# Qualcomm-AI-research/FP8-quantization

Measured on AMD Instinct MI355X. Metric: FP8 quant+dequant Gelems/sec, higher is better.
Workload: dtype f32; 1 GPU; conv1-shaped weights [2097152,3,7,7] fp32 per GPU, per-channel E5M2 quantize+dequantize, fixed ranges from current_minmax (BASELINE config 2, synthetic NxCxKxK scale-up); elements_per_gpu=308281344, parallelism=1 GPU

## Files before the change

fp8-quantization_amd/csrc/fp8q_common.h:

```cpp
#pragma once
#include <hip/hip_runtime.h>
#include <math.h>

#include <atomic>
#include <stdint.h>
#include <stdio.h>
#include <stdlib.h>
#include <string.h>

#include <climits>
#include <type_traits>

#include "../../include/fp8q.h"
#include "fp8q_device.h"

using namespace fp8q;

constexpr int FP8Q_CODEC_NOT_FLAT = -1000;
int fp8q_codec_flat_launch(bool encode, const void *in, void *out, int64_t C, int64_t inner, const float *maxval,
                           const QFmt &f, int n_bits, hipStream_t st);

namespace {

constexpr int kUnroll = 4;
constexpr int kTargetBlocks = 2048;
constexpr int kDirectMaxInner = 16384;
constexpr int kDirectElems = 32768;
static const int64_t kNtBytes = [] {
    const char *e = getenv("FP8Q_NT_MB");
    const long v = e ? atol(e) : 0;
    return (int64_t)(v >= 1 ? v : 64) << 20;
}();

inline int env_int(const char *name, int dflt, int lo = INT_MIN, int hi = INT_MAX)
{
    const char *e = getenv(name);
    if (!e) return dflt;
    const long v = atol(e);
    return v < lo ? lo : (v > hi ? hi : (int)v);
}

template <auto V>
using Const = std::integral_constant<decltype(V), V>;
// ... 233 lines not shown
```

fp8-quantization_amd/csrc/fp8q_quant.hip:

```cpp
#include "fp8q_rows.h"
#include "fp8q_select.h"

namespace {

template <bool NT, int U>
__device__ __forceinline__ void quant_rows_body(const float *__restrict__ x, float *__restrict__ y, int64_t inner,
                                                const float *__restrict__ maxval, int per_channel, const QFmt &f)
{
    __shared__ float2 lut[kLutMax];
    const int row = blockIdx.y;
    const int tid = threadIdx.x;
    const Chan cfull = make_chan(maxval[per_channel ? row : 0], f);
    for (int i = tid; i <= f.pmax; i += kBlock) lut[i] = lut_entry(cfull, i, f.M);
    __syncthreads();
    const ChanLite c = lite(cfull);
    const float pmaxf = (float)f.pmax;
    const float qthr = f.qthr;

    const float *xr = x + (int64_t)row * inner;
    float *yr = y + (int64_t)row * inner;
    int64_t head = ((16 - ((uintptr_t)xr & 15)) & 15) >> 2;
    if (head > inner) head = inner;
    const int64_t nvec = (inner - head) >> 2;
    const int64_t tail0 = head + (nvec << 2);
// ... 202 lines not shown
    for (int64_t row = (int64_t)blockIdx.x * (kBlock / 64) + wave; row < C; row += (int64_t)gridDim.x * (kBlock / 64)) {
        const Chan cfull = make_chan(maxval[row], f);
        for (int i = lane; i <= f.pmax; i += 64) lut[wave][i] = lut_entry(cfull, i, f.M);
        __builtin_amdgcn_wave_barrier();
        const ChanLite c = lite(cfull);
        const float *xr = x + row * inner;
        float *yr = y + row * inner;
        for (int i = lane; i < inner; i += 64) yr[i] = quant_one(xr[i], c, lut[wave], pmaxf, f.qthr);
        __builtin_amdgcn_wave_barrier();
    }
}

template <class SEL>
__global__ void __launch_bounds__(kBlock)
k_quant_scalar_dm(const float *__restrict__ x, float *__restrict__ y, int64_t inner, const float *__restrict__ maxval,
                  int per_channel, SEL sel)
{
    const QFmt f = pick_fmt(sel);
    quant_scalar_body(x, y, inner, maxval, per_channel, f);
}

template <bool NT>
__global__ void __launch_bounds__(kBlock)
k_copy(const vf4 *__restrict__ x, vf4 *__restrict__ y, int64_t nvec)
{
    const int tid = threadIdx.x;
    const int64_t step = (int64_t)gridDim.x * (kBlock * kUnroll);
    for (int64_t base = (int64_t)blockIdx.x * (kBlock * kUnroll); base < nvec; base += step) {
        if (base + kBlock * kUnroll <= nvec) {
            vf4 v[kUnroll];
#pragma unroll
            for (int u = 0; u < kUnroll; ++u) v[u] = ld16<NT>(x + base + u * kBlock + tid);
#pragma unroll
            for (int u = 0; u < kUnroll; ++u) st16<NT>(y + base + u * kBlock + tid, v[u]);
        } else {
            for (int u = 0; u < kUnroll; ++u) {
                const int64_t i = base + u * kBlock + tid;
                if (i < nvec) st16<NT>(y + i, ld16<NT>(x + i));
            }
        }
    }
}

struct RowGrid {
    bool nt;
    bool small;
    int64_t bx;
    int64_t bs;
};

constexpr int64_t kSmallElems = (int64_t)8 << 20;

inline int64_t k1_total_cap(bool nt, int64_t pieces, int64_t big_cap = 65536)
{
    return (!nt || pieces <= 4096) ? kTargetBlocks : big_cap;
}

template <class CapRule>
RowGrid row_grid(int64_t C, int64_t inner, int64_t small_elems, CapRule total_cap, bool partial_piece = false)
{
    RowGrid g;
// ... 190 lines not shown
    const bool aligned = (((uintptr_t)x ^ (uintptr_t)y) & 15) == 0 && ((uintptr_t)x & 3) == 0;
    if (!aligned) return FP8Q_EUNSUPPORTED;
    SelIn si;
    si.mses = mses;
    si.grid = grid;
    si.n_m = n_m;
    si.n_cand = n_cand;
    si.so = *so;
    static const int64_t sel_cap = getenv("FP8Q_SEL_CAP") ? atoll(getenv("FP8Q_SEL_CAP")) : kTargetBlocks;
    const RowGrid g = row_grid(1, n, kSmallElems, [](bool nt, int64_t pieces) { return k1_total_cap(nt, pieces, sel_cap); });
    dispatch_k1(g, [&](auto NT, auto U) {
        hipLaunchKernelGGL((k_quant_rows_sel<NT(), U()>), dim3((unsigned)g.bx, 1u), dim3(kBlock), 0, st, x, y, n, sel, si);
    });
    return launch_rc();
}

extern "C" {

int fp8q_copy_f32(const float *x, float *y, int64_t n, fp8q_stream_t stream)
{
    if (!x || !y || n < 0 || (n & 3) || ((uintptr_t)x & 15) || ((uintptr_t)y & 15)) return FP8Q_EINVAL;
    if (n == 0) return FP8Q_OK;
    const RowGrid g = row_grid(1, n, 0, [](bool, int64_t pieces) { return (int64_t)(pieces > 4096 ? 65536 : kTargetBlocks); }, true);
    dispatch<true, false>(g.nt, [&](auto NT) {
        hipLaunchKernelGGL(k_copy<NT()>, dim3((unsigned)g.bx), dim3(kBlock), 0, (hipStream_t)stream, (const vf4 *)x, (vf4 *)y, n / 4);
    });
    return launch_rc();
}

}
```

fp8-quantization_amd/csrc/fp8q_rows.h:

```cpp
#pragma once
#include "fp8q_common.h"

namespace {

constexpr int kModeQuant = 0, kModeFused = 1, kModeMinMax = 2;
constexpr int kModeEncode = 3, kModeDecode = 4;

struct TileArgs {
    int inner;
    int rows;
    int lut_stride;
    int group;
    int coaligned;
    uint32_t magic;
    uint32_t lmagic;
};

__device__ __forceinline__ ChanLite lite_lds(const Chan *c)
{
    const float4 h = *reinterpret_cast<const float4 *>(c);
    ChanLite l;
    l.maxv = h.x;
    l.minv = h.y;
    l.bias = h.z;
    l.pthr = h.w;
    return l;
}

constexpr int kChunkElems = 4096, kChunkGroups = 1024, kFlatMaxCh = 8;
constexpr int kFlatFusedMaxInner = 256;

struct FlatArgs {
    int inner;
    int rpc;
    int nch;
    int lut_stride;
    int group;
    int tail;
    uint32_t magic;
    uint32_t rmagic;
    int64_t nvec;
    int64_t nchunks;
    int n_bits;
    int pad0;
};

struct __attribute__((aligned(16))) ChunkInfo {
    int64_t row_lo;
    int phase;
    int nrows;
    int len;
    int tail;
    int pad[2];
};

__device__ __forceinline__ int64_t div_rows(int64_t elo, int inner)
{
    int64_t q = (int64_t)((double)elo / (double)inner);
    int64_t r = elo - q * inner;
    if (r < 0) --q, r += inner;
    if (r >= inner) ++q;
    return q;
}

constexpr int kNotFlat = -1000;
static_assert(kNotFlat == FP8Q_CODEC_NOT_FLAT, "fp8q_codec_flat_launch passes the code through");

inline int64_t flat_rpc(int64_t inner) { return (inner + (kChunkElems + 3) - 2) / inner + 1; }

inline int64_t flat_per_row(int lut_stride, bool fused = false) { return 16 + 16 + (int64_t)lut_stride * 8 + (fused ? 4 : 0); }

inline FlatArgs flat_geometry(int64_t C, int64_t inner, int lut_stride)
{
    FlatArgs a = {};
    a.inner = (int)inner;
    a.lut_stride = lut_stride;
    a.magic = magic_of((int)inner);
    const int64_t n = C * inner;
    a.nvec = n >> 2;
    a.tail = (int)(n & 3);
    a.nchunks = cdiv(a.nvec, kChunkGroups);
    a.rpc = (int)flat_rpc(inner);
    a.rmagic = magic_of(a.rpc);
    return a;
}

}

#define FP8Q_HIDDEN extern "C" __attribute__((visibility("hidden")))
FP8Q_HIDDEN int64_t fp8q_direct_max_inner();
FP8Q_HIDDEN int fp8q_launch_rows_direct(int mode, const float *x, float *y, int64_t C, int64_t inner, const float *maxval,
                                   float *row_min, float *row_max, float *maxval_out, const QFmt &f, const FoldArgs &fa,
                                   hipStream_t st);
FP8Q_HIDDEN int fp8q_launch_rows_reg(bool quant, const float *x, float *y, int64_t C, int64_t inner, float *row_min, float *row_max,
                                float *maxval_out, const QFmt &f, const FoldArgs &fa, hipStream_t st);
FP8Q_HIDDEN int fp8q_launch_rows_staged_mm(const float *x, int64_t C, int64_t inner, float *row_min, float *row_max,
                                      float *maxval_out, const FoldArgs &fa, hipStream_t st);
```

fp8-quantization_amd/csrc/fp8q_rows.hip:

```cpp
#include "fp8q_rows.h"

namespace {

template <int MODE, bool LUT, bool NT>
__global__ void __launch_bounds__(kBlock, 4)
k_rows_direct(const float *__restrict__ x, float *__restrict__ y, int64_t C,
              const float *__restrict__ maxval, float *row_min, float *row_max, float *maxval_out,
              QFmt f, TileArgs a, FoldArgs fa)
{
    extern __shared__ __attribute__((aligned(16))) unsigned char smem[];
    const int Rmax = a.rows;
    float *rowmv = reinterpret_cast<float *>(smem);
    float4 *patch = reinterpret_cast<float4 *>(rowmv + ((Rmax + 3) & ~3));
    Chan *chans = reinterpret_cast<Chan *>(patch + Rmax);
    float2 *lut = reinterpret_cast<float2 *>(chans + Rmax);
    const int tid = threadIdx.x;
    constexpr int BS = kBlock;
    const int G = a.group, rpp = BS / G;
    const int sub = tid & (G - 1), slot = tid / G;
    const int inner = a.inner, inner4 = inner & ~3;
    const float pmaxf = (float)f.pmax;
    __shared__ double ftab_lds[kFastTabSize];
    const double *ftab = ftab_lds;
    if (MODE != kModeMinMax)
// ... 100 lines not shown
                    const int ch = div_small((uint32_t)o, a.magic);
                    const int b = inner - (o - ch * inner);
                    float e[4] = {v[u].x, v[u].y, v[u].z, v[u].w};
                    if (LUT) {
                        quant_group<4>(e, lite_lds(chans + ch), lut + ch * a.lut_stride, pmaxf, f.qthr);
                    } else {
                        const Chan c = chans[ch];
#pragma unroll
                        for (int q = 0; q < 4; ++q) e[q] = quant_direct(e[q], c, f.M);
                    }
                    if (b < 4) {
                        const float4 pt = patch[ch];
                        e[3] = b == 3 ? pt.x : (b == 2 ? pt.y : pt.z);
                        if (b < 3) e[2] = b == 2 ? pt.x : pt.y;
                        if (b < 2) e[1] = pt.x;
                    }
                    st16u<NT>(yt + o, vf4{e[0], e[1], e[2], e[3]});
                }
            }
        }
    }
}

template <int MODE, bool NT>
__global__ void __launch_bounds__(kBlock, 4)
k_rows_flat(const float *__restrict__ x, float *__restrict__ y, const float *__restrict__ maxval,
            float *row_min, float *row_max, float *maxval_out, QFmt f, FlatArgs a)
{
    extern __shared__ __attribute__((aligned(16))) unsigned char smem[];
    __shared__ double ftab[kFastTabSize];
    const int Rt = a.rpc * a.nch;
    ChunkInfo *cinfo = reinterpret_cast<ChunkInfo *>(smem);
    float4 *patch = reinterpret_cast<float4 *>(cinfo + kFlatMaxCh);
    float4 *chl = patch + Rt;
    float2 *lut = reinterpret_cast<float2 *>(chl + Rt);
    float *rowmv = reinterpret_cast<float *>(lut + Rt * a.lut_stride);
    const int tid = threadIdx.x;
    const int inner = a.inner;
    const int64_t G = gridDim.x;
    const float pmaxf = (float)f.pmax;
    for (int i = tid; i < kFastTabSize; i += kBlock) ftab[i] = kFastTab[i];

    for (int64_t c0 = blockIdx.x; c0 < a.nchunks; c0 += G * a.nch) {
        int nct = 1;
        while (nct < a.nch && c0 + nct * G < a.nchunks) ++nct;
        const int nlr = nct * a.rpc;
        __syncthreads();
        if (tid < nct) {
            const int64_t c = c0 + tid * G;
            const int64_t elo = c * kChunkElems;
            const int64_t rem = a.nvec * 4 - elo;
            ChunkInfo ci;
            ci.len = rem < kChunkElems ? (int)rem : kChunkElems;
            ci.tail = (c == a.nchunks - 1) ? a.tail : 0;
            ci.row_lo = elo / inner;
            ci.phase = (int)(elo - ci.row_lo * inner);
            ci.nrows = (ci.phase + ci.len + ci.tail - 1) / inner + 1;
            ci.pad[0] = ci.pad[1] = 0;
            cinfo[tid] = ci;
        }
        __syncthreads();
        if (MODE == kModeFused) {
            const int Gl = a.group, rpp = kBlock / Gl, sub = tid & (Gl - 1), slot = tid / Gl;
            const int inner4 = inner & ~3;
            for (int lrb = 0; lrb < nlr; lrb += rpp) {
                const int lr = lrb + slot;
                const int i = div_small((uint32_t)lr, a.rmagic), r = lr - i * a.rpc;
                const bool valid = lr < nlr && r < cinfo[i].nrows;
                MinMax m;
                mm_init(m);
                if (valid) {
                    const float *xr = x + (cinfo[i].row_lo + r) * inner;
                    int j = sub * 4;
                    for (; j + 3 * Gl * 4 < inner4; j += Gl * 16) {
                        vf4 v[4];
#pragma unroll
                        for (int u = 0; u < 4; ++u) v[u] = ld16u<false>(xr + j + u * Gl * 4);
#pragma unroll
                        for (int u = 0; u < 4; ++u) {
                            mm_acc(m, v[u].x);
                            mm_acc(m, v[u].y);
                            mm_acc(m, v[u].z);
                            mm_acc(m, v[u].w);
                        }
// ... 157 lines not shown
                const int o = phase + 4 * q;
                const int lrow = div_small((uint32_t)o, a.magic);
                const int b = inner - (o - lrow * inner);
                const int lr = lr0 + lrow;
                float e[4] = {v[u].x, v[u].y, v[u].z, v[u].w};
                quant_group<4>(e, lite_of(chl[lr]), lut + lr * a.lut_stride, pmaxf, f.qthr);
                if (b < 4) {
                    const float4 pt = patch[lr];
                    e[3] = b == 3 ? pt.x : (b == 2 ? pt.y : pt.z);
                    if (b < 3) e[2] = b == 2 ? pt.x : pt.y;
                    if (b < 2) e[1] = pt.x;
                }
                st16<NT>(yv + q, vf4{e[0], e[1], e[2], e[3]});
            }
        }
    }
}

constexpr int kStagePad = 256;
constexpr int kStageWin = kStagePad + kChunkElems + kStagePad;
constexpr size_t kStageMaxLds = 36 * 1024;
constexpr int kStageGrid = 2048;
static_assert(kStagePad >= kFlatFusedMaxInner - 1 && kStagePad % 4 == 0, "border rows must fit the pads");

__device__ __forceinline__ ChunkInfo stage_geometry(int64_t c, const FlatArgs &a)
{
    ChunkInfo ci;
    const int64_t elo = c * kChunkElems;
    const int64_t rem = a.nvec * 4 - elo;
    ci.len = rem < kChunkElems ? (int)rem : kChunkElems;
    ci.tail = (c == a.nchunks - 1) ? a.tail : 0;
    ci.row_lo = div_rows(elo, a.inner);
    ci.phase = (int)(elo - ci.row_lo * a.inner);
    ci.nrows = div_small((uint32_t)(ci.phase + ci.len + ci.tail - 1), a.magic) + 1;
    ci.pad[0] = ci.nrows * a.inner - ci.phase - ci.len;
    ci.pad[1] = 0;
    return ci;
}

__device__ __forceinline__ ChunkInfo stage_geometry_next(const ChunkInfo &cur, int64_t cn, uint32_t adv, const FlatArgs &a)
{
    ChunkInfo ci;
    const int64_t elo = cn * kChunkElems;
    const int64_t rem = a.nvec * 4 - elo;
    ci.len = rem < kChunkElems ? (int)rem : kChunkElems;
    ci.tail = (cn == a.nchunks - 1) ? a.tail : 0;
    const uint32_t t = (uint32_t)cur.phase + adv;
    const uint32_t q = (uint32_t)div_small(t, a.magic);
    ci.row_lo = cur.row_lo + q;
    ci.phase = (int)(t - q * (uint32_t)a.inner);
    ci.nrows = div_small((uint32_t)(ci.phase + ci.len + ci.tail - 1), a.magic) + 1;
    ci.pad[0] = ci.nrows * a.inner - ci.phase - ci.len;
    ci.pad[1] = 0;
    return ci;
}

constexpr int kStageU = 4;

template <bool NT>
__device__ __forceinline__ void stage_load_body(const float *x, int64_t c, const FlatArgs &a, vf4 (&v)[kStageU])
{
// ... 250 lines not shown

}

int64_t fp8q_direct_max_inner()
{
    static const int v = [] {
        const char *e = getenv("FP8Q_DIRECT_MAX_INNER");
        const int n = e ? atoi(e) : 0;
        return n >= 4 && n <= kDirectMaxInner ? n : 2047;
    }();
    return v;
}

static int64_t flat_nch(const FlatArgs &a, int64_t per_row, int64_t lds_bytes, int64_t max_nch)
{
    int64_t nch = (lds_bytes - (int64_t)kFlatMaxCh * sizeof(ChunkInfo)) / (a.rpc * per_row);
    if (nch > max_nch) nch = max_nch;
    while (nch > 1 && cdiv(a.nchunks, nch) < 1024) --nch;
    return nch;
}

static size_t flat_shmem(const FlatArgs &a, int64_t per_row) { return (size_t)kFlatMaxCh * sizeof(ChunkInfo) + (size_t)a.rpc * a.nch * per_row; }

static int launch_rows_flat(int mode, const float *x, float *y, int64_t C, int64_t inner, const float *maxval,
                            float *row_min, float *row_max, float *maxval_out, const QFmt &f, hipStream_t st)
{
    static const int flat_env = env_int("FP8Q_FLAT", 1);
    if (!flat_env || mode == kModeMinMax || inner < 4) return kNotFlat;
    if ((((uintptr_t)x | (uintptr_t)y) & 15) != 0) return kNotFlat;
    if (mode == kModeFused && (inner > kFlatFusedMaxInner || x == y)) return kNotFlat;
    FlatArgs a = flat_geometry(C, inner, f.pmax + 1);
    const int64_t per_row = flat_per_row(a.lut_stride, mode == kModeFused);
    static const int lds_kb_env = [] {
        const char *e = getenv("FP8Q_FLAT_LDS_KB");
        const int v = e ? atoi(e) : 0;
        return v >= 4 && v <= 120 ? v : 36;
    }();
    static const int nch_env = [] {
        const char *e = getenv("FP8Q_FLAT_NCH");
        const int v = e ? atoi(e) : 0;
        return v >= 1 && v <= kFlatMaxCh ? v : 4;
    }();
    const int64_t nch = flat_nch(a, per_row, (int64_t)lds_kb_env * 1024, nch_env);
    if (nch < 1) return kNotFlat;
    const bool nt = C * inner * 4 >= kNtBytes;
    if (mode == kModeFused) {
        static const int staged_env = env_int("FP8Q_STAGED", 1);
        static const int staged_grid = [] {
            const char *e = getenv("FP8Q_STAGED_GRID");
            const int v = e ? atoi(e) : -1;
            return v >= 0 ? v : kStageGrid;
        }();
        const size_t sh = (size_t)kStageWin * sizeof(float) + (size_t)a.rpc * per_row;
        if (staged_env && sh <= kStageMaxLds) {
            int gs = 0;
            while (gs < 6 && (2 << gs) * a.rpc <= kBlock) ++gs;
            a.group = gs;
            a.nch = 1;
            const int64_t blocks = staged_grid ? balanced_blocks(a.nchunks, staged_grid) : a.nchunks;
            dispatch<true, false>(nt, [&](auto NT) {
                hipLaunchKernelGGL((k_rows_staged<NT()>), dim3((unsigned)blocks), dim3(kBlock), sh, st, x, y, row_min, row_max,
                                   maxval_out, f, a);
            });
            return launch_rc();
        }
    }
    a.nch = (int)nch;
    int G = 1;
    while (G < 64 && (int64_t)G * 24 < inner) G <<= 1;
    a.group = G;
    static const int grid_env = env_int("FP8Q_FLAT_GRID", 0, 0);
    int64_t blocks = cdiv(a.nchunks, a.nch);
    const int64_t grid_cap = grid_env ? grid_env : ((mode == kModeQuant && a.nchunks <= 16384) ? 1024 : 32768);
    if (blocks > grid_cap) blocks = grid_cap;
    dispatch<kModeQuant, kModeFused>(mode, [&](auto MODE) {
        dispatch<true, false>(nt, [&](auto NT) {
            hipLaunchKernelGGL((k_rows_flat<MODE(), NT()>), dim3((unsigned)blocks), dim3(kBlock), flat_shmem(a, per_row), st, x, y,
                               maxval, row_min, row_max, maxval_out, f, a);
        });
    });
    return launch_rc();
}

__attribute__((visibility("hidden"))) int fp8q_codec_flat_launch(bool encode, const void *in, void *out, int64_t C,
                                                                 int64_t inner, const float *maxval, const QFmt &f,
                                                                 int n_bits, hipStream_t st)
{
    const void *fp = encode ? in : (const void *)out;
    const void *cp = encode ? (const void *)out : in;
    if (inner < 4 || inner > fp8q_direct_max_inner() || ((uintptr_t)fp & 15) != 0 || ((uintptr_t)cp & 3) != 0) return kNotFlat;
    FlatArgs a = flat_geometry(C, inner, f.pmax + 1);
    a.n_bits = n_bits;
    const int64_t per_row = flat_per_row(a.lut_stride);
    const int64_t nch = flat_nch(a, per_row, 36 * 1024, 4);
    if (nch < 1) return kNotFlat;
    a.nch = (int)nch;
    a.group = 1;
    int64_t blocks = cdiv(a.nchunks, nch);
    if (blocks > 32768) blocks = 32768;
    const bool nt = C * inner * 4 >= kNtBytes;
    const float *xf = (const float *)in;
    float *yf = (float *)out;
    dispatch<kModeEncode, kModeDecode>(encode ? kModeEncode : kModeDecode, [&](auto MODE) {
        dispatch<true, false>(nt, [&](auto NT) {
            hipLaunchKernelGGL((k_rows_flat<MODE(), NT()>), dim3((unsigned)blocks), dim3(kBlock), flat_shmem(a, per_row), st, xf, yf,
                               maxval, nullptr, nullptr, nullptr, f, a);
        });
    });
    return launch_rc();
}

int fp8q_launch_rows_staged_mm(const float *x, int64_t C, int64_t inner, float *row_min, float *row_max, float *maxval_out,
                          const FoldArgs &fa, hipStream_t st)
{
    static const int staged_env = env_int("FP8Q_STAGED", 1);
    if (!staged_env || inner < 4 || inner > kFlatFusedMaxInner || ((uintptr_t)x & 15) != 0) return kNotFlat;
    FlatArgs a = flat_geometry(C, inner, 0);
    int gs = 0;
    while (gs < 3 && (2 << gs) * a.rpc <= kBlock) ++gs;
    a.group = gs;
    static const int grid_env = env_int("FP8Q_STAGED_MM_GRID", 0, 0);
    const int64_t blocks = grid_env ? balanced_blocks(a.nchunks, grid_env) : a.nchunks;
    dispatch<true, false>(C * inner * 4 >= kNtBytes, [&](auto NT) {
        hipLaunchKernelGGL((k_rows_staged_mm<NT()>), dim3((unsigned)blocks), dim3(kBlock), 0, st, x, row_min, row_max, maxval_out,
                           fa, a);
    });
// ... 49 lines not shown
    static const int mm_blocks_env = env_int("FP8Q_K2_BLOCKS", 65536);
    const int64_t bcap = mode == kModeMinMax ? mm_blocks_env : 2 * kTargetBlocks;
    if (blocks > bcap) blocks = balanced_blocks(blocks, bcap);
    const bool nt = C * inner * 4 >= kNtBytes;
    const dim3 g((unsigned)blocks), b(BSZ);
    auto launch = [&](auto MODE, auto LUT, auto NT) {
        hipLaunchKernelGGL((k_rows_direct<MODE(), LUT(), NT()>), g, b, shmem, st, x, y, C, maxval, row_min, row_max,
                           maxval_out, f, a, fa);
    };
    if (mode == kModeMinMax) {
        launch(Const<kModeMinMax>{}, Const<false>{}, Const<false>{});
    } else {
        dispatch<kModeQuant, kModeFused>(mode, [&](auto MODE) {
            dispatch<true, false>(lut, [&](auto LUT) { dispatch<true, false>(nt, [&](auto NT) { launch(MODE, LUT, NT); }); });
        });
    }
    return launch_rc();
}

extern "C" {

int64_t fp8q_fused_max_inner(void) { return kDirectMaxInner; }

int fp8q_minmax_quantize_f32(const float *x, float *y, int64_t C, int64_t inner, float *row_min,
                             float *row_max, float *maxval_out, float mbits, int n_bits,
                             int sign_bits, fp8q_stream_t stream)
{
    if (C < 0 || inner < 0) return FP8Q_EINVAL;
    QFmt f;
    if (int rc = make_fmt(mbits, n_bits, sign_bits, &f)) return rc;
    if (C == 0 || inner == 0) return FP8Q_OK;
    if (!x || !y) return FP8Q_EINVAL;
    if (inner > kDirectMaxInner) return FP8Q_ETOOLONG;
    if (((uintptr_t)x & 3) != 0 || ((uintptr_t)y & 3) != 0) return FP8Q_EINVAL;
    hipStream_t st = (hipStream_t)stream;
    static const bool small_fused = env_int("FP8Q_SMALL_FUSED", 1) != 0;
    const FoldArgs nofold = {0, 1, 0.0f, 0.0f};
    if (small_fused && C * inner <= kSmallFusedElems && inner <= kSmallFusedInner) {
        dispatch<1, 2, 3, 4, 8>((int)cdiv(inner, 64), [&](auto EPL) {
            hipLaunchKernelGGL(k_small_rows_fused<EPL()>, dim3((unsigned)cdiv(C, kBlock / 64)), dim3(kBlock), 0, st, x, y, C,
                               (int)inner, row_min, row_max, maxval_out, f);
        });
        return launch_rc();
    }
    const int rc = fp8q_launch_rows_reg(true, x, y, C, inner, row_min, row_max, maxval_out, f, nofold, st);
    if (rc != kNotFlat) return rc;
// ... 5 lines not shown
```

fp8-quantization_amd/fp8q/_lib.py:

```python
import ctypes
import os

from . import build as _build

_lib = None

_i64 = ctypes.c_int64
_vp = ctypes.c_void_p
_f = ctypes.c_float
_i = ctypes.c_int



class MseState(ctypes.Structure):
    _fields_ = [("cur_min", _vp), ("cur_max", _vp), ("absmax", _vp), ("grid", _vp), ("mses", _vp), ("maxval", _vp),
                ("xmin", _vp), ("mbits", _vp), ("vote", _vp)]


class MseRouteInfo(ctypes.Structure):
    _fields_ = [("kernel", _i), ("finish", _i), ("nsplit", _i64), ("tiles_per_wg", _i), ("part_wgs", _i), ("slice_min", _i),
                ("moments_threads", _i), ("n_superblocks", _i64), ("top_scan", _i), ("reserved", _i)]


class AffinePre(ctypes.Structure):
    _fields_ = [("x", _vp), ("residual", _vp), ("alpha_beta", _vp), ("N", _i64), ("C", _i64), ("HW", _i64), ("act", _i)]


class AffineRouteInfo(ctypes.Structure):
    _fields_ = [("kernel", _i), ("direct", _i), ("cpp", _i), ("launches", _i), ("grid_x", _i64), ("grid_y", _i64)]


class MxtRouteInfo(ctypes.Structure):
    _fields_ = [("kernel", _i), ("tile_rows", _i), ("tile_cols", _i), ("nontemporal", _i), ("code_store_bytes", _i),
                ("reserved", _i)]


class TensorDesc(ctypes.Structure):
    _fields_ = [("x", _vp), ("y", _vp), ("maxval", _vp), ("C", _i64), ("inner", _i64), ("n_maxval", _i64),
                ("mbits", _f), ("n_bits", _i), ("sign_bits", _i)]


SIGNATURES = {
    "fp8q_version": (_i, []),
    "fp8q_strerror": (ctypes.c_char_p, [_i]),
    "fp8q_quantize_f32": (_i, [_vp, _vp, _i64, _i64, _vp, _i64, _f, _i, _i, _vp]),
    "fp8q_minmax_workspace_bytes": (ctypes.c_size_t, [_i64, _i64]),
    "fp8q_minmax_f32": (_i, [_vp, _i64, _i64, _vp, _vp, _vp, _i, ctypes.c_double, _i, _vp,
                             ctypes.c_size_t, _vp]),
    "fp8q_minmax_packed_f32": (_i, [_vp, _i64, _i64, _vp, _vp, _vp, _vp, _i, ctypes.c_double, _i, _vp,
                                    ctypes.c_size_t, _vp]),
    "fp8q_ranges_unpack_f32": (_i, [_vp, _i64, _vp, _vp, _vp, _vp]),
    "fp8q_minmax_workspace_check": (_i, [_vp, ctypes.c_size_t, _i, _vp]),
    "fp8q_fused_max_inner": (_i64, []),
    "fp8q_minmax_quantize_f32": (_i, [_vp, _vp, _i64, _i64, _vp, _vp, _vp, _f, _i, _i, _vp]),
    "fp8q_mse_workspace_bytes": (ctypes.c_size_t, [_i64, _i64, _i64, _i]),
    "fp8q_mse_grid_f32": (_i, [_vp, _i64, _i64, _vp, _i64, ctypes.POINTER(_f), _i, _i, _i, _vp, _vp,
                               ctypes.c_size_t, _vp]),
# ... 24 lines not shown
    "fp8q_quantizer_prepare_f32": (_i, [_vp, _f, _i, _i, _vp, _vp]),
    "fp8q_affine_act_quantize_ab_f32": (_i, [_vp, _vp, _vp, _i64, _i64, _i64, _vp, _i, _vp, _vp, _f, _i, _i, _vp]),
    "fp8q_affine_act_f32": (_i, [_vp, _vp, _vp, _i64, _i64, _i64, _vp, _i, _vp]),
    "fp8q_affine_act_route": (_i, [_i64, _i64, _i64, _i, ctypes.POINTER(AffineRouteInfo)]),
    "fp8q_affine_act_minmax_linspace_f32": (_i, [_vp, _vp, _vp, _i64, _i64, _i64, _vp, _i, _vp, _vp, _vp, _vp, _i, ctypes.c_double,
                                                 ctypes.c_double, _vp, ctypes.c_size_t, _vp]),
    "fp8q_affine_act_minmax_workspace_bytes": (ctypes.c_size_t, [_i64, _i64, _i64]),
    "fp8q_affine_act_minmax_f32": (_i, [_vp, _vp, _i64, _i64, _i64, _vp, _vp, _vp, _vp, _i, _vp, _vp, _vp, _i,
                                        ctypes.c_double, _i, _vp, ctypes.c_size_t, _vp]),
    "fp8q_affine_act_minmax_packed_f32": (_i, [_vp, _vp, _i64, _i64, _i64, _vp, _vp, _vp, _vp, _i, _vp, _vp, _vp, _vp,
                                               _i, ctypes.c_double, _i, _vp, ctypes.c_size_t, _vp]),
    "fp8q_encode_u8": (_i, [_vp, _vp, _i64, _i64, _vp, _i64, _f, _i, _i, _vp]),
    "fp8q_decode_u8": (_i, [_vp, _vp, _i64, _i64, _vp, _i64, _f, _i, _i, _vp]),
    "fp8q_multi_quantize_f32": (_i, [ctypes.POINTER(TensorDesc), _i, _vp]),
    "fp8q_multi_minmax_quantize_f32": (_i, [ctypes.POINTER(TensorDesc), ctypes.POINTER(_vp), _i, _vp]),
    "fp8q_multi_encode_u8": (_i, [ctypes.POINTER(TensorDesc), _i, _vp]),
    "fp8q_multi_minmax_encode_u8": (_i, [ctypes.POINTER(TensorDesc), ctypes.POINTER(_vp), _i, _vp]),
    "fp8q_multi_decode_u8": (_i, [ctypes.POINTER(TensorDesc), _i, _vp]),
    "fp8q_multi_plan_create": (_i, [ctypes.POINTER(TensorDesc), _i, ctypes.POINTER(_vp)]),
    "fp8q_multi_plan_launch": (_i, [_vp, _vp]),
    "fp8q_multi_plan_launches": (_i, [_vp]),
    "fp8q_multi_plan_destroy": (None, [_vp]),
    "fp8q_copy_f32": (_i, [_vp, _vp, _i64, _vp]),
    "fp8q_int_quantize_f32": (_i, [_vp, _vp, _i64, _i64, _vp, _vp, _i64, _vp, _i, _i, _f, _vp]),
    "fp8q_int_set_range_f32": (_i, [_vp, _vp, _i64, _vp, _vp, _vp, _i, _i, _f, _vp]),
    "fp8q_int_range_quantize_f32": (_i, [_vp, _vp, _i64, _i64, _vp, _vp, _i64, _vp, _vp, _vp, _i, _i, _f, _vp]),
    "fp8q_int_minmax_quantize_f32": (_i, [_vp, _vp, _i64, _i64, _vp, _vp, _vp, _vp, _vp, _i, _i, _f, _vp,
                                          ctypes.c_size_t, _vp]),
    "fp8q_int_affine_act_quantize_f32": (_i, [_vp, _vp, _vp, _i64, _i64, _i64, _vp, _i, _vp, _vp, _vp, _i, _i, _f, _vp]),
    "fp8q_int_affine_act_range_quantize_f32": (_i, [_vp, _vp, _vp, _i64, _i64, _i64, _vp, _i, _vp, _vp, _vp, _vp, _vp, _i, _i,
                                                    _f, _vp]),
    "fp8q_int_sse_grid_workspace_bytes": (ctypes.c_size_t, [_i64, _i64, _i64]),
    "fp8q_int_sse_grid_f32": (_i, [_vp, _i64, _i64, _vp, _i64, _i, _i, _i, _f, _vp, _vp, ctypes.c_size_t, _vp]),
    "fp8q_int_sse_grid_f64": (_i, [_vp, _i64, _i64, _vp, _i64, _i, _i, _i, _f, _vp, _vp, ctypes.c_size_t, _vp]),
    "fp8q_quantize_h16": (_i, [_vp, _vp, _i, _i, _i64, _i64, _vp, _i64, _f, _i, _i, _vp]),
    "fp8q_minmax_h16": (_i, [_vp, _i, _i64, _i64, _vp, _vp, _vp, _i, ctypes.c_double, _i, _vp, ctypes.c_size_t, _vp]),
    "fp8q_minmax_quantize_h16": (_i, [_vp, _vp, _i, _i, _i64, _i64, _vp, _vp, _vp, _f, _i, _i, _vp]),
    "fp8q_int_quantize_h16": (_i, [_vp, _vp, _i, _i, _i64, _i64, _vp, _vp, _i64, _vp, _i, _i, _f, _vp]),
    "fp8q_int_range_quantize_h16": (_i, [_vp, _vp, _i, _i, _i64, _i64, _vp, _vp, _i64, _vp, _vp, _vp, _i, _i, _f, _vp]),
    "fp8q_int_minmax_quantize_h16": (_i, [_vp, _vp, _i, _i, _i64, _i64, _vp, _vp, _vp, _vp, _vp, _i, _i, _f, _vp,
                                          ctypes.c_size_t, _vp]),
    "fp8q_encode_h16": (_i, [_vp, _vp, _i, _i64, _i64, _vp, _i64, _f, _i, _i, _vp]),
    "fp8q_decode_h16": (_i, [_vp, _vp, _i, _i64, _i64, _vp, _i64, _f, _i, _i, _vp]),
    "fp8q_int_encode_h16": (_i, [_vp, _vp, _i, _i64, _i64, _vp, _vp, _i64, _vp, _i, _i, _f, _vp]),
    "fp8q_int_decode_h16": (_i, [_vp, _vp, _i, _i64, _i64, _vp, _vp, _i64, _vp, _i, _i, _f, _vp]),
    "fp8q_quantize_bwd_f32": (_i, [_vp, _vp, _vp, _i64, _i64, _vp, _i64, _f, _vp, _i, _i, _vp, _vp, _vp, ctypes.c_size_t, _vp]),
# ... 63 lines not shown
```

fp8-quantization_amd/fp8q/ops.py:

```python
import torch

from ._lib import Fp8qError, check, lib

FOLD_CURRENT, FOLD_ALL, FOLD_RUNNING = 0, 1, 2

_ws_cache = {}
_ws_retired = []
_mm_ws_bytes = {}


_raw_stream = getattr(torch._C, "_cuda_getCurrentRawStream", None)


def _stream(t):
    if _raw_stream is not None:
        return _raw_stream(t.device.index)
    return torch.cuda.current_stream(t.device).cuda_stream


class _on_device:
    __slots__ = ("idx", "prev")

    def __init__(self, t):
        self.idx = t.device.index
# ... 882 lines not shown
        if tuple(out.shape) != (n_cand, C) or not out.is_contiguous():
            raise Fp8qError(f"out must be contiguous [{n_cand}, {C}]")
    L = lib()
    ws = _workspace(x.device, L.fp8q_int_sse_grid_workspace_bytes(C, inner, n_cand))
    fn, name = ((L.fp8q_int_sse_grid_f64, "fp8q_int_sse_grid_f64") if x.dtype == torch.float64
                else (L.fp8q_int_sse_grid_f32, "fp8q_int_sse_grid_f32"))
    with _on_device(x):
        rc = fn(x.data_ptr(), C, inner, thr.data_ptr(), n_cand, int(n_bits), int(bool(symmetric)), int(bool(one_sided)),
                float(eps), out.data_ptr(), ws.data_ptr(), ws.numel(), _stream(x))
    check(rc, name)
    return out


def copy(x, out=None):
    _require(x, "x")
    x = x.contiguous()
    y = _out(out, x)
    with _on_device(x):
        rc = lib().fp8q_copy_f32(x.data_ptr(), y.data_ptr(), x.numel(), _stream(x))
    check(rc, "fp8q_copy_f32")
    return y


_mse_ws_bytes = {}


def mse_grid(x, per_channel, grid, mbits_list, n_bits, sign_bits, mses):
    import ctypes
    _require(x, "x")
    _require(grid, "grid", like=x)
    _require(mses, "mses", like=x)
    flat = None if per_channel else _dense_flat(x)
    x = flat if flat is not None else x.contiguous()
    C, inner = _rows(x, per_channel)
    n_m = len(mbits_list)
    n_cand = grid.shape[0]
    if grid.dim() != 2 or grid.shape[1] != C or not grid.is_contiguous():
        raise Fp8qError(f"grid must be contiguous [n_cand, {C}]")
    if tuple(mses.shape) != (n_m, n_cand, C) or not mses.is_contiguous():
        raise Fp8qError(f"mses must be contiguous [{n_m}, {n_cand}, {C}]")
    L = lib()
    key = (C, inner, n_cand, n_m)
    nbytes = _mse_ws_bytes.get(key)
    if nbytes is None:
        nbytes = _mse_ws_bytes[key] = L.fp8q_mse_workspace_bytes(C, inner, n_cand, n_m)
    ws = _workspace(x.device, nbytes)
# ... 805 lines not shown
```

include/fp8q.h:

```cpp
#ifndef FP8Q_H
#define FP8Q_H

#include <stddef.h>
#include <stdint.h>

#ifdef __cplusplus
extern "C" {
#endif

#define FP8Q_VERSION 601

#define FP8Q_OK 0
#define FP8Q_EINVAL (-1)
#define FP8Q_EUNSUPPORTED (-2)
#define FP8Q_EWORKSPACE (-3)
#define FP8Q_ETOOLONG (-4)
#define FP8Q_ETOOMANY (-5)
#define FP8Q_ETIMEDOUT (-6)

#define FP8Q_FOLD_CURRENT 0
#define FP8Q_FOLD_ALL 1
#define FP8Q_FOLD_RUNNING 2


// ... 146 lines not shown
typedef struct fp8q_tensor_desc {
    const float *x;
    float *y;
    const float *maxval;
    int64_t C, inner, n_maxval;
    float mbits;
    int n_bits, sign_bits;
} fp8q_tensor_desc;
int fp8q_multi_quantize_f32(const fp8q_tensor_desc *descs, int n, fp8q_stream_t stream);

int fp8q_multi_minmax_quantize_f32(const fp8q_tensor_desc *descs, float *const *maxval_out, int n, fp8q_stream_t stream);
int fp8q_multi_encode_u8(const fp8q_tensor_desc *descs, int n, fp8q_stream_t stream);
int fp8q_multi_minmax_encode_u8(const fp8q_tensor_desc *descs, float *const *maxval_out, int n, fp8q_stream_t stream);
int fp8q_multi_decode_u8(const fp8q_tensor_desc *descs, int n, fp8q_stream_t stream);

typedef struct fp8q_multi_plan fp8q_multi_plan;
int fp8q_multi_plan_create(const fp8q_tensor_desc *descs, int n, fp8q_multi_plan **plan);
int fp8q_multi_plan_launch(const fp8q_multi_plan *plan, fp8q_stream_t stream);
int fp8q_multi_plan_launches(const fp8q_multi_plan *plan);
void fp8q_multi_plan_destroy(fp8q_multi_plan *plan);

int fp8q_copy_f32(const float *x, float *y, int64_t n, fp8q_stream_t stream);

int fp8q_int_quantize_f32(const float *x, float *y, int64_t C, int64_t inner, const float *delta,
                          const float *zero_float, int64_t n_delta, const unsigned char *signed_flag, int n_bits,
                          int symmetric, float eps, fp8q_stream_t stream);
int fp8q_int_set_range_f32(const float *x_min, const float *x_max, int64_t n, float *delta, float *zero_float,
                           unsigned char *signed_flag, int n_bits, int symmetric, float eps, fp8q_stream_t stream);
int fp8q_int_range_quantize_f32(const float *x, float *y, int64_t C, int64_t inner, const float *x_min,
                                const float *x_max, int64_t n_range, float *delta, float *zero_float,
                                unsigned char *signed_flag, int n_bits, int symmetric, float eps,
                                fp8q_stream_t stream);
int fp8q_int_minmax_quantize_f32(const float *x, float *y, int64_t C, int64_t inner, float *row_min, float *row_max,
                                 float *delta, float *zero_float, unsigned char *signed_flag, int n_bits, int symmetric,
                                 float eps, void *ws, size_t ws_bytes, fp8q_stream_t stream);

int fp8q_int_affine_act_quantize_f32(const float *x, const float *residual, float *y, int64_t N, int64_t C, int64_t HW,
                                     const float *alpha_beta, int act, const float *delta, const float *zero_float,
                                     const unsigned char *signed_flag, int n_bits, int symmetric, float eps,
                                     fp8q_stream_t stream);
int fp8q_int_affine_act_range_quantize_f32(const float *x, const float *residual, float *y, int64_t N, int64_t C, int64_t HW,
                                           const float *alpha_beta, int act, const float *x_min, const float *x_max,
                                           float *delta_out, float *zero_float_out, unsigned char *signed_flag_out, int n_bits,
                                           int symmetric, float eps, fp8q_stream_t stream);

int fp8q_int_to_integer_f32(const float *x, float *t, int64_t C, int64_t inner, const float *delta,
// ... 129 lines not shown
```

Baseline: 763.4 Gelem/s.

## Add windowed chunk-tile scheduling for flat row kernels and copy

Introduces a FlatTile scheduler that can group chunks into occupancy-sized windows so that concurrently resident blocks touch nearby memory, and applies it to k_rows_flat, the codec kernels and k_copy. The window defaults to off (0) unless FP8Q_FLAT_WINDOW is set, so the default path keeps the old strided assignment. The per-chunk geometry staging now uses the magic-division helper, and a wave barrier replaces a block barrier. It also adds a route-query API for inspecting the chosen kernel and grid.

Result: no change. 759.1 Gelem/s (-0.6%).

```diff
diff --git a/fp8-quantization_amd/csrc/fp8q_common.h b/fp8-quantization_amd/csrc/fp8q_common.h
--- a/fp8-quantization_amd/csrc/fp8q_common.h
+++ b/fp8-quantization_amd/csrc/fp8q_common.h
@@ -18,7 +18,7 @@
 
 constexpr int FP8Q_CODEC_NOT_FLAT = -1000;
 int fp8q_codec_flat_launch(bool encode, const void *in, void *out, int64_t C, int64_t inner, const float *maxval,
-                           const QFmt &f, int n_bits, hipStream_t st);
+                           const QFmt &f, int n_bits, hipStream_t st, fp8q_rows_flat_route_info *route = nullptr);
 
 namespace {
 
diff --git a/fp8-quantization_amd/csrc/fp8q_quant.hip b/fp8-quantization_amd/csrc/fp8q_quant.hip
--- a/fp8-quantization_amd/csrc/fp8q_quant.hip
+++ b/fp8-quantization_amd/csrc/fp8q_quant.hip
@@ -248,21 +248,24 @@
 
 template <bool NT>
 __global__ void __launch_bounds__(kBlock)
-k_copy(const vf4 *__restrict__ x, vf4 *__restrict__ y, int64_t nvec)
+k_copy(const vf4 *__restrict__ x, vf4 *__restrict__ y, int64_t nvec, int64_t npieces, int64_t ntiles, int nch, int W)
 {
     const int tid = threadIdx.x;
-    const int64_t step = (int64_t)gridDim.x * (kBlock * kUnroll);
-    for (int64_t base = (int64_t)blockIdx.x * (kBlock * kUnroll); base < nvec; base += step) {
-        if (base + kBlock * kUnroll <= nvec) {
-            vf4 v[kUnroll];
-#pragma unroll
-            for (int u = 0; u < kUnroll; ++u) v[u] = ld16<NT>(x + base + u * kBlock + tid);
-#pragma unroll
-            for (int u = 0; u < kUnroll; ++u) st16<NT>(y + base + u * kBlock + tid, v[u]);
-        } else {
-            for (int u = 0; u < kUnroll; ++u) {
-                const int64_t i = base + u * kBlock + tid;
-                if (i < nvec) st16<NT>(y + i, ld16<NT>(x + i));
+    FlatTile tile;
+    for (int64_t it = 0; flat_tile(it, npieces, ntiles, nch, W, tile); ++it) {
+        for (int i = 0; i < tile.n; ++i) {
+            const int64_t base = (tile.c0 + i * tile.stride) * (kBlock * kUnroll);
+            if (base + kBlock * kUnroll <= nvec) {
+                vf4 v[kUnroll];
+#pragma unroll
+                for (int u = 0; u < kUnroll; ++u) v[u] = ld16<NT>(x + base + u * kBlock + tid);
+#pragma unroll
+                for (int u = 0; u < kUnroll; ++u) st16<NT>(y + base + u * kBlock + tid, v[u]);
+            } else {
+                for (int u = 0; u < kUnroll; ++u) {
+                    const int64_t j = base + u * kBlock + tid;
+                    if (j < nvec) st16<NT>(y + j, ld16<NT>(x + j));
+                }
             }
         }
     }
@@ -499,8 +502,19 @@
     if (!x || !y || n < 0 || (n & 3) || ((uintptr_t)x & 15) || ((uintptr_t)y & 15)) return FP8Q_EINVAL;
     if (n == 0) return FP8Q_OK;
     const RowGrid g = row_grid(1, n, 0, [](bool, int64_t pieces) { return (int64_t)(pieces > 4096 ? 65536 : kTargetBlocks); }, true);
+    const int64_t pieces = cdiv(n / 4, kBlock * kUnroll);
+    int W = 0;
+    if (pieces > 16384)
+        dispatch<true, false>(g.nt, [&](auto NT) {
+            W = fp8q_flat_window(reinterpret_cast<const void *>(&k_copy<NT()>), NT() ? 15 : 14, 0);
+        });
+    if (W < 0) return hip_rc((hipError_t)-W);
+    const int nch = W > 0 ? 4 : 1;
+    const int64_t ntiles = flat_tile_count(pieces, nch, W);
+    const int64_t blocks = W > 0 ? (ntiles < 32768 ? ntiles : 32768) : g.bx;
     dispatch<true, false>(g.nt, [&](auto NT) {
-        hipLaunchKernelGGL(k_copy<NT()>, dim3((unsigned)g.bx), dim3(kBlock), 0, (hipStream_t)stream, (const vf4 *)x, (vf4 *)y, n / 4);
+        hipLaunchKernelGGL(k_copy<NT()>, dim3((unsigned)blocks), dim3(kBlock), 0, (hipStream_t)stream, (const vf4 *)x, (vf4 *)y, n / 4,
+                           pieces, ntiles, nch, W);
     });
     return launch_rc();
 }
diff --git a/fp8-quantization_amd/csrc/fp8q_rows.h b/fp8-quantization_amd/csrc/fp8q_rows.h
--- a/fp8-quantization_amd/csrc/fp8q_rows.h
+++ b/fp8-quantization_amd/csrc/fp8q_rows.h
@@ -42,7 +42,8 @@
     int64_t nvec;
     int64_t nchunks;
     int n_bits;
-    int pad0;
+    int window;
+    int64_t ntiles;
 };
 
 struct __attribute__((aligned(16))) ChunkInfo {
@@ -61,6 +62,44 @@
     if (r < 0) --q, r += inner;
     if (r >= inner) ++q;
     return q;
+}
+
+inline int64_t flat_tile_count(int64_t nchunks, int nch, int W)
+{
+    if (W <= 0) return (nchunks + nch - 1) / nch;
+    const int64_t per = (int64_t)W * nch;
+    return (nchunks / per) * W + (nchunks % per + nch - 1) / nch;
+}
+
+struct FlatTile {
+    int64_t c0;
+    int64_t stride;
+    int n;
+};
+
+__device__ __forceinline__ bool flat_tile(int64_t it, int64_t nchunks, int64_t ntiles, int nch, int W, FlatTile &t)
+{
+    const int64_t G = gridDim.x;
+    int64_t left;
+    if (W <= 0) {
+        t.c0 = blockIdx.x + it * G * nch;
+        if (t.c0 >= nchunks) return false;
+        t.stride = G;
+        left = nchunks - t.c0;
+    } else {
+        const int64_t T = blockIdx.x + it * G;
+        if (T >= ntiles) return false;
+        const int64_t w = (uint64_t)T < (1ull << 32) ? (int64_t)((uint32_t)T / (uint32_t)W) : T / W;
+        const int64_t j = T - w * W, base = w * W * nch;
+        const int64_t per = (int64_t)W * nch;
+        const int64_t nw = nchunks - base < per ? nchunks - base : per;
+        t.stride = nw < per ? (int64_t)(((uint32_t)nw + (uint32_t)nch - 1u) / (uint32_t)nch) : W;
+        t.c0 = base + j;
+        left = nw - j;
+    }
+    t.n = 1;
+    while (t.n < nch && t.n * t.stride < left) ++t.n;
+    return true;
 }
 
 constexpr int kNotFlat = -1000;
@@ -89,6 +128,7 @@
 
 #define FP8Q_HIDDEN extern "C" __attribute__((visibility("hidden")))
 FP8Q_HIDDEN int64_t fp8q_direct_max_inner();
+FP8Q_HIDDEN int fp8q_flat_window(const void *kernel, int slot, size_t shmem);
 FP8Q_HIDDEN int fp8q_launch_rows_direct(int mode, const float *x, float *y, int64_t C, int64_t inner, const float *maxval,
                                    float *row_min, float *row_max, float *maxval_out, const QFmt &f, const FoldArgs &fa,
                                    hipStream_t st);
diff --git a/fp8-quantization_amd/csrc/fp8q_rows.hip b/fp8-quantization_amd/csrc/fp8q_rows.hip
--- a/fp8-quantization_amd/csrc/fp8q_rows.hip
+++ b/fp8-quantization_amd/csrc/fp8q_rows.hip
@@ -146,6 +146,21 @@
     }
 }
 
+__device__ __forceinline__ ChunkInfo stage_geometry(int64_t c, const FlatArgs &a)
+{
+    ChunkInfo ci;
+    const int64_t elo = c * kChunkElems;
+    const int64_t rem = a.nvec * 4 - elo;
+    ci.len = rem < kChunkElems ? (int)rem : kChunkElems;
+    ci.tail = (c == a.nchunks - 1) ? a.tail : 0;
+    ci.row_lo = div_rows(elo, a.inner);
+    ci.phase = (int)(elo - ci.row_lo * a.inner);
+    ci.nrows = div_small((uint32_t)(ci.phase + ci.len + ci.tail - 1), a.magic) + 1;
+    ci.pad[0] = ci.nrows * a.inner - ci.phase - ci.len;
+    ci.pad[1] = 0;
+    return ci;
+}
+
 template <int MODE, bool NT>
 __global__ void __launch_bounds__(kBlock, 4)
 k_rows_flat(const float *__restrict__ x, float *__restrict__ y, const float *__restrict__ maxval,
@@ -161,29 +176,19 @@
     float *rowmv = reinterpret_cast<float *>(lut + Rt * a.lut_stride);
     const int tid = threadIdx.x;
     const int inner = a.inner;
-    const int64_t G = gridDim.x;
     const float pmaxf = (float)f.pmax;
     for (int i = tid; i < kFastTabSize; i += kBlock) ftab[i] = kFastTab[i];
 
-    for (int64_t c0 = blockIdx.x; c0 < a.nchunks; c0 += G * a.nch) {
-        int nct = 1;
-        while (nct < a.nch && c0 + nct * G < a.nchunks) ++nct;
+    FlatTile tile;
+    for (int64_t it = 0; flat_tile(it, a.nchunks, a.ntiles, a.nch, a.window, tile); ++it) {
+        const int64_t c0 = tile.c0, G = tile.stride;
+        const int nct = tile.n;
         const int nlr = nct * a.rpc;
         __syncthreads();
-        if (tid < nct) {
-            const int64_t c = c0 + tid * G;
-            const int64_t elo = c * kChunkElems;
-            const int64_t rem = a.nvec * 4 - elo;
-            ChunkInfo ci;
-            ci.len = rem < kChunkElems ? (int)rem : kChunkElems;
-            ci.tail = (c == a.nchunks - 1) ? a.tail : 0;
-            ci.row_lo = elo / inner;
-            ci.phase = (int)(elo - ci.row_lo * inner);
-            ci.nrows = (ci.phase + ci.len + ci.tail - 1) / inner + 1;
-            ci.pad[0] = ci.pad[1] = 0;
-            cinfo[tid] = ci;
-        }
-        __syncthreads();
+        if ((tid & 63) < nct) cinfo[tid & 63] = stage_geometry(c0 + (tid & 63) * G, a);
+        __builtin_amdgcn_fence(__ATOMIC_RELEASE, "wavefront");
+        __builtin_amdgcn_wave_barrier();
+        __builtin_amdgcn_fence(__ATOMIC_ACQUIRE, "wavefront");
         if (MODE == kModeFused) {
             const int Gl = a.group, rpp = kBlock / Gl, sub = tid & (Gl - 1), slot = tid / Gl;
             const int inner4 = inner & ~3;
@@ -387,21 +392,6 @@
 constexpr size_t kStageMaxLds = 36 * 1024;
 constexpr int kStageGrid = 2048;
 static_assert(kStagePad >= kFlatFusedMaxInner - 1 && kStagePad % 4 == 0, "border rows must fit the pads");
-
-__device__ __forceinline__ ChunkInfo stage_geometry(int64_t c, const FlatArgs &a)
-{
-    ChunkInfo ci;
-    const int64_t elo = c * kChunkElems;
-    const int64_t rem = a.nvec * 4 - elo;
-    ci.len = rem < kChunkElems ? (int)rem : kChunkElems;
-    ci.tail = (c == a.nchunks - 1) ? a.tail : 0;
-    ci.row_lo = div_rows(elo, a.inner);
-    ci.phase = (int)(elo - ci.row_lo * a.inner);
-    ci.nrows = div_small((uint32_t)(ci.phase + ci.len + ci.tail - 1), a.magic) + 1;
-    ci.pad[0] = ci.nrows * a.inner - ci.phase - ci.len;
-    ci.pad[1] = 0;
-    return ci;
-}
 
 __device__ __forceinline__ ChunkInfo stage_geometry_next(const ChunkInfo &cur, int64_t cn, uint32_t adv, const FlatArgs &a)
 {
@@ -698,8 +688,68 @@
 
 static size_t flat_shmem(const FlatArgs &a, int64_t per_row) { return (size_t)kFlatMaxCh * sizeof(ChunkInfo) + (size_t)a.rpc * a.nch * per_row; }
 
+constexpr int kFlatMaxWindow = 1 << 20;
+constexpr bool kFlatWindowDefault = false;
+
+int fp8q_flat_window(const void *kernel, int slot, size_t shmem)
+{
+    static const int env = env_int("FP8Q_FLAT_WINDOW", kFlatWindowDefault ? -1 : 0, -1, kFlatMaxWindow);
+    if (env >= 0) return env;
+    struct Seen {
+        int dev = -1, w = 0;
+        size_t shmem = 0;
+    };
+    thread_local Seen seen[16];
+    Seen &s = seen[slot];
+    int dev = 0;
+    if (hipError_t e = hipGetDevice(&dev)) return -(int)e;
+    if (s.dev != dev || s.shmem != shmem) {
+        int cus = 0, per_cu = 0;
+        if (hipError_t e = hipDeviceGetAttribute(&cus, hipDeviceAttributeMultiprocessorCount, dev)) return -(int)e;
+        if (hipError_t e = hipOccupancyMaxActiveBlocksPerMultiprocessor(&per_cu, kernel, kBlock, shmem)) return -(int)e;
+        const int64_t w = (int64_t)cus * per_cu;
+        s.w = w < 1 ? 1 : (w > kFlatMaxWindow ? kFlatMaxWindow : (int)w);
+        s.dev = dev;
+        s.shmem = shmem;
+    }
+    return s.w;
+}
+
+template <int MODE, bool NT>
+static int flat_window_of(size_t shmem)
+{
+    return fp8q_flat_window(reinterpret_cast<const void *>(&k_rows_flat<MODE, NT>), MODE * 2 + (NT ? 1 : 0), shmem);
+}
+
+static int flat_tiles(int mode, bool nt, bool windowed, size_t shmem, int64_t grid_cap, FlatArgs &a, int64_t *blocks)
+{
+    int w = 0;
+    if (windowed)
+        dispatch<kModeQuant, kModeFused, kModeEncode, kModeDecode>(mode, [&](auto MODE) {
+            dispatch<true, false>(nt, [&](auto NT) { w = flat_window_of<MODE(), NT()>(shmem); });
+        });
+    if (w < 0) return hip_rc((hipError_t)-w);
+    a.window = w;
+    a.ntiles = flat_tile_count(a.nchunks, a.nch, w);
+    *blocks = a.ntiles < grid_cap ? a.ntiles : grid_cap;
+    return FP8Q_OK;
+}
+
+static void flat_report(fp8q_rows_flat_route_info *r, int kernel, const FlatArgs &a, int64_t blocks, bool nt)
+{
+    r->kernel = kernel;
+    r->nch = a.nch;
+    r->rpc = a.rpc;
+    r->window = a.window;
+    r->nontemporal = nt;
+    r->nchunks = a.nchunks;
+    r->ntiles = a.ntiles;
+    r->grid = blocks;
+}
+
 static int launch_rows_flat(int mode, const float *x, float *y, int64_t C, int64_t inner, const float *maxval,
-                            float *row_min, float *row_max, float *maxval_out, const QFmt &f, hipStream_t st)
+                            float *row_min, float *row_max, float *maxval_out, const QFmt &f, hipStream_t st,
+                            fp8q_rows_flat_route_info *route = nullptr)
 {
     static const int flat_env = env_int("FP8Q_FLAT", 1);
     if (!flat_env || mode == kModeMinMax || inner < 4) return kNotFlat;
@@ -734,6 +784,11 @@
             a.group = gs;
             a.nch = 1;
             const int64_t blocks = staged_grid ? balanced_blocks(a.nchunks, staged_grid) : a.nchunks;
+            if (route) {
+                a.ntiles = a.nchunks;
+                flat_report(route, FP8Q_ROWS_STAGED, a, blocks, nt);
+                return FP8Q_OK;
+            }
             dispatch<true, false>(nt, [&](auto NT) {
                 hipLaunchKernelGGL((k_rows_staged<NT()>), dim3((unsigned)blocks), dim3(kBlock), sh, st, x, y, row_min, row_max,
                                    maxval_out, f, a);
@@ -746,9 +801,14 @@
     while (G < 64 && (int64_t)G * 24 < inner) G <<= 1;
     a.group = G;
     static const int grid_env = env_int("FP8Q_FLAT_GRID", 0, 0);
-    int64_t blocks = cdiv(a.nchunks, a.nch);
-    const int64_t grid_cap = grid_env ? grid_env : ((mode == kModeQuant && a.nchunks <= 16384) ? 1024 : 32768);
-    if (blocks > grid_cap) blocks = grid_cap;
+    const bool resident = mode == kModeQuant && a.nchunks <= 16384;
+    const int64_t grid_cap = grid_env ? grid_env : (resident ? 1024 : 32768);
+    int64_t blocks = 0;
+    if (int rc = flat_tiles(mode, nt, !resident, flat_shmem(a, per_row), grid_cap, a, &blocks)) return rc;
+    if (route) {
+        flat_report(route, FP8Q_ROWS_FLAT, a, blocks, nt);
+        return FP8Q_OK;
+    }
     dispatch<kModeQuant, kModeFused>(mode, [&](auto MODE) {
         dispatch<true, false>(nt, [&](auto NT) {
             hipLaunchKernelGGL((k_rows_flat<MODE(), NT()>), dim3((unsigned)blocks), dim3(kBlock), flat_shmem(a, per_row), st, x, y,
@@ -760,7 +820,8 @@
 
 __attribute__((visibility("hidden"))) int fp8q_codec_flat_launch(bool encode, const void *in, void *out, int64_t C,
                                                                  int64_t inner, const float *maxval, const QFmt &f,
-                                                                 int n_bits, hipStream_t st)
+                                                                 int n_bits, hipStream_t st,
+                                                                 fp8q_rows_flat_route_info *route)
 {
     const void *fp = encode ? in : (const void *)out;
     const void *cp = encode ? (const void *)out : in;
@@ -772,12 +833,17 @@
     if (nch < 1) return kNotFlat;
     a.nch = (int)nch;
     a.group = 1;
-    int64_t blocks = cdiv(a.nchunks, nch);
-    if (blocks > 32768) blocks = 32768;
     const bool nt = C * inner * 4 >= kNtBytes;
+    const int mode = encode ? kModeEncode : kModeDecode;
+    int64_t blocks = 0;
+    if (int rc = flat_tiles(mode, nt, true, flat_shmem(a, per_row), 32768, a, &blocks)) return rc;
+    if (route) {
+        flat_report(route, FP8Q_ROWS_FLAT, a, blocks, nt);
+        return FP8Q_OK;
+    }
     const float *xf = (const float *)in;
     float *yf = (float *)out;
-    dispatch<kModeEncode, kModeDecode>(encode ? kModeEncode : kModeDecode, [&](auto MODE) {
+    dispatch<kModeEncode, kModeDecode>(mode, [&](auto MODE) {
         dispatch<true, false>(nt, [&](auto NT) {
             hipLaunchKernelGGL((k_rows_flat<MODE(), NT()>), dim3((unsigned)blocks), dim3(kBlock), flat_shmem(a, per_row), st, xf, yf,
                                maxval, nullptr, nullptr, nullptr, f, a);
@@ -873,6 +939,26 @@
 
 int64_t fp8q_fused_max_inner(void) { return kDirectMaxInner; }
 
+int fp8q_rows_flat_route(int mode, int64_t C, int64_t inner, float mbits, int n_bits, int sign_bits,
+                         fp8q_rows_flat_route_info *info)
+{
+    if (!info || C < 1 || inner < 1 || (mode != kModeQuant && mode != kModeFused && mode != kModeEncode && mode != kModeDecode))
+        return FP8Q_EINVAL;
+    QFmt f;
+    if (int rc = make_fmt(mbits, n_bits, sign_bits, &f)) return rc;
+    *info = {};
+    const float *x = reinterpret_cast<const float *>((uintptr_t)4096);
+    float *y = reinterpret_cast<float *>((uintptr_t)8192);
+    int rc = kNotFlat;
+    if (inner <= fp8q_direct_max_inner()) {
+        if (mode == kModeEncode || mode == kModeDecode)
+            rc = fp8q_codec_flat_launch(mode == kModeEncode, x, y, C, inner, nullptr, f, n_bits, nullptr, info);
+        else
+            rc = launch_rows_flat(mode, x, y, C, inner, nullptr, nullptr, nullptr, nullptr, f, nullptr, info);
+    }
+    return rc == kNotFlat ? FP8Q_OK : rc;
+}
+
 int fp8q_minmax_quantize_f32(const float *x, float *y, int64_t C, int64_t inner, float *row_min,
                              float *row_max, float *maxval_out, float mbits, int n_bits,
                              int sign_bits, fp8q_stream_t stream)
diff --git a/fp8-quantization_amd/fp8q/_lib.py b/fp8-quantization_amd/fp8q/_lib.py
--- a/fp8-quantization_amd/fp8q/_lib.py
+++ b/fp8-quantization_amd/fp8q/_lib.py
@@ -33,6 +33,11 @@
 class MxtRouteInfo(ctypes.Structure):
     _fields_ = [("kernel", _i), ("tile_rows", _i), ("tile_cols", _i), ("nontemporal", _i), ("code_store_bytes", _i),
                 ("reserved", _i)]
+
+
+class RowsFlatRouteInfo(ctypes.Structure):
+    _fields_ = [("kernel", _i), ("nch", _i), ("rpc", _i), ("window", _i), ("nontemporal", _i), ("reserved", _i),
+                ("nchunks", _i64), ("ntiles", _i64), ("grid", _i64)]
 
 
 class TensorDesc(ctypes.Structure):
@@ -103,6 +108,7 @@
     "fp8q_multi_plan_launches": (_i, [_vp]),
     "fp8q_multi_plan_destroy": (None, [_vp]),
     "fp8q_copy_f32": (_i, [_vp, _vp, _i64, _vp]),
+    "fp8q_rows_flat_route": (_i, [_i, _i64, _i64, _f, _i, _i, ctypes.POINTER(RowsFlatRouteInfo)]),
     "fp8q_int_quantize_f32": (_i, [_vp, _vp, _i64, _i64, _vp, _vp, _i64, _vp, _i, _i, _f, _vp]),
     "fp8q_int_set_range_f32": (_i, [_vp, _vp, _i64, _vp, _vp, _vp, _i, _i, _f, _vp]),
     "fp8q_int_range_quantize_f32": (_i, [_vp, _vp, _i64, _i64, _vp, _vp, _i64, _vp, _vp, _vp, _i, _i, _f, _vp]),
diff --git a/fp8-quantization_amd/fp8q/ops.py b/fp8-quantization_amd/fp8q/ops.py
--- a/fp8-quantization_amd/fp8q/ops.py
+++ b/fp8-quantization_amd/fp8q/ops.py
@@ -928,6 +928,18 @@
     return y
 
 
+def rows_flat_route(op, C, inner, mbits, n_bits=8, sign_bits=1):
+    import ctypes
+    from ._lib import RowsFlatRouteInfo
+    info = RowsFlatRouteInfo()
+    mode = {"quantize": 0, "minmax_quantize": 1, "encode": 3, "decode": 4}[op]
+    check(lib().fp8q_rows_flat_route(mode, int(C), int(inner), float(mbits), int(n_bits), int(sign_bits), ctypes.byref(info)),
+          "fp8q_rows_flat_route")
+    r = {name: int(getattr(info, name)) for name, _ in RowsFlatRouteInfo._fields_ if name != "reserved"}
+    r["kernel"] = ("other", "flat", "staged")[r["kernel"]]
+    return r
+
+
 _mse_ws_bytes = {}
 
 
diff --git a/include/fp8q.h b/include/fp8q.h
--- a/include/fp8q.h
+++ b/include/fp8q.h
@@ -192,6 +192,21 @@
 
 int fp8q_copy_f32(const float *x, float *y, int64_t n, fp8q_stream_t stream);
 
+#define FP8Q_ROWS_OTHER 0
+#define FP8Q_ROWS_FLAT 1
+#define FP8Q_ROWS_STAGED 2
+typedef struct fp8q_rows_flat_route_info {
+    int kernel;
+    int nch;
+    int rpc;
+    int window;
+    int nontemporal;
+    int reserved;
+    int64_t nchunks, ntiles, grid;
+} fp8q_rows_flat_route_info;
+int fp8q_rows_flat_route(int mode, int64_t C, int64_t inner, float mbits, int n_bits, int sign_bits,
+                         fp8q_rows_flat_route_info *info);
+
 int fp8q_int_quantize_f32(const float *x, float *y, int64_t C, int64_t inner, const float *delta,
                           const float *zero_float, int64_t n_delta, const unsigned char *signed_flag, int n_bits,
                           int symmetric, float eps, fp8q_stream_t stream);
```
